# KatherLab/STAMP

Measured on AMD Instinct MI355X. Metric: tiles/sec encoded (224x224, ViT-L/14), higher is better.
Workload: dtype f16

## Files before the change

include/amdstamp.h:

```cpp
#ifndef AMDSTAMP_H
#define AMDSTAMP_H

#include <stddef.h>
#include <stdint.h>

#ifdef __cplusplus
extern "C" {
#endif

#define AMDS_VERSION_MAJOR 0
#define AMDS_VERSION_MINOR 2

typedef enum {
    AMDS_OK = 0,
    AMDS_ERR_INVALID = -1,
    AMDS_ERR_WORKSPACE = -2,
    AMDS_ERR_HIP = -3,
    AMDS_ERR_NODEVICE = -4,
    AMDS_ERR_RANGE = -5
} amds_status;

typedef enum { AMDS_F16 = 0, AMDS_BF16 = 1, AMDS_F32 = 2 } amds_dtype;

typedef enum {
// ... 145 lines not shown

typedef struct {
    const void*  patch_w;
    const float* patch_b;
    const float* prefix;
    const float* pos_patch;
    const amds_vit_block* blocks_host;
    const float* norm_w; const float* norm_b;
    int patch_lo_shift;
    const amds_vit_exact_block* exact_host;
    int exact_hidden;
    const amds_vit_fp8_block* fp8_host;
    const float* pre_norm_w;
    const float* pre_norm_b;
    const amds_vit_exact_block* cls_tail;
} amds_vit_weights;

typedef struct {
    const float* norm1_w; const float* norm1_b;
    const float* qkv_w;   const float* qkv_b;
    const float* proj_w;  const float* proj_b;
    const float* ls1;
    const float* norm2_w; const float* norm2_b;
    const float* fc1_w;   const float* fc1_b;
    const float* fc2_w;   const float* fc2_b;
    const float* ls2;
} amds_vit_host_block;
typedef struct {
    const float* patch_w;
    const float* patch_b;
// ... 24 lines not shown
int amds_vit_forward(const amds_vit_cfg* cfg_host, const amds_vit_weights* w_host,
                     const uint8_t* tiles, void* feats_f16, int B, int chunk,
                     void* ws, size_t ws_bytes, void* stream);

int amds_check_finite(const void* x, long n, int dtype, int* count_dev, int* count_host, void* stream);

int amds_vit_forward_tokens(const amds_vit_cfg* cfg_host, const amds_vit_weights* w_host,
                            const uint8_t* tiles, void* feats_f16, float* tokens_f32, int B, int chunk,
                            void* ws, size_t ws_bytes, void* stream);

int amds_vit_forward_overlapped(amds_ctx* ctx, const amds_vit_cfg* cfg_host, const amds_vit_weights* w_host, const uint8_t* tiles,
                                void* feats_f16, int B, int chunk, void* ws, size_t ws_bytes, void* stream);

int amds_attention_cls_f32(const float* q, long ldq, const void* qkv, float* out, long ldo, int B, int T, int H, int head_dim,
                           int dtype, void* stream);
int amds_vit_cls_gather(const float* x, float* xc, int B, int T, int D, void* stream);
int amds_vit_cls_scatter(const float* xc, float* x, void* xh, float* rowstat, int B, int T, int D, float eps, int dtype, void* stream);
int amds_mlp_act_f32(float* u, long ld, int rows, int hidden, int kind, void* stream);

int amds_tile_im2col_u8(const uint8_t* tiles, void* out, int B, int img, int patch, int kp,
                        int dtype, void* stream);
int amds_tile_im2col_u8_ex(const uint8_t* tiles, void* out, int B, int img, int patch, int kp,
                           int dtype, int lo_shift, void* stream);

int amds_tile_normalize_u8(const uint8_t* hwc, float* chw, int B, int H, int W,
                           const float mean_host[3], const float std_host[3], void* stream);

int amds_tile_edge_fraction_u8(const uint8_t* tiles, float* frac, uint8_t* edges, uint8_t* gray, int B, int S, int low, int high,
                               void* stream);

// ... 647 lines not shown
```

stamp_amd/_lib.py:

```python
from __future__ import annotations

import ctypes as C
import os
from pathlib import Path

LIB_PATH = Path(__file__).resolve().parent / "lib" / "libamdstamp.so"

F16, BF16, F32 = 0, 1, 2
ERR_RANGE = -5
(EPI_BIAS, EPI_BIAS_GELU, EPI_BIAS_RELU, EPI_RESIDUAL, EPI_BIAS_F32, EPI_SWIGLU, EPI_PATCH,
 EPI_BIAS_GELU_F32, EPI_BIAS_RELU_F32) = range(9)


class VitCfg(C.Structure):
    _fields_ = [("img", C.c_int), ("patch", C.c_int), ("dim", C.c_int), ("depth", C.c_int),
                ("heads", C.c_int), ("hidden", C.c_int), ("n_prefix", C.c_int), ("mlp_kind", C.c_int),
                ("layerscale", C.c_int), ("dtype", C.c_int), ("ln_eps", C.c_float)]


class VitBlock(C.Structure):
    _fields_ = [(n, C.c_void_p) for n in (
        "ln1_w", "ln1_b", "qkv_w", "qkv_b", "proj_w", "proj_b", "ls1",
        "ln2_w", "ln2_b", "fc1_w", "fc1_b", "fc2_w", "fc2_b", "ls2", "qkv_colsum", "fc1_colsum")]


class VitExactBlock(C.Structure):
    _fields_ = [(n, C.c_void_p) for n in ("q_w", "q_b", "proj_w", "proj_b", "fc1_w", "fc1_b", "fc2_w", "fc2_b")]


class VitFp8Block(C.Structure):
    _fields_ = ([(n, C.c_void_p) for n in ("qkv_w8", "qkv_cs", "proj_w8", "proj_cs", "proj_b", "fc1_w8", "fc1_cs")] + [("fc1_wnorm_max", C.c_float), ("fc1_babs_max", C.c_float)]
                + [(n, C.c_void_p) for n in ("fc2_w8", "fc2_cs", "fc2_b")])


class VitWeights(C.Structure):
    _fields_ = [("patch_w", C.c_void_p), ("patch_b", C.c_void_p), ("prefix", C.c_void_p),
                ("pos_patch", C.c_void_p), ("blocks_host", C.POINTER(VitBlock)),
                ("norm_w", C.c_void_p), ("norm_b", C.c_void_p), ("patch_lo_shift", C.c_int),
                ("exact_host", C.POINTER(VitExactBlock)), ("exact_hidden", C.c_int), ("fp8_host", C.POINTER(VitFp8Block)),
                ("pre_norm_w", C.c_void_p), ("pre_norm_b", C.c_void_p), ("cls_tail", C.POINTER(VitExactBlock))]


class VitHostBlock(C.Structure):
    _fields_ = [(n, C.c_void_p) for n in ("norm1_w", "norm1_b", "qkv_w", "qkv_b", "proj_w", "proj_b", "ls1", "norm2_w", "norm2_b",
                                          "fc1_w", "fc1_b", "fc2_w", "fc2_b", "ls2")]


class VitHostWeights(C.Structure):
    _fields_ = [("patch_w", C.c_void_p), ("patch_b", C.c_void_p), ("cls_token", C.c_void_p), ("reg_token", C.c_void_p), ("pos_embed", C.c_void_p),
                ("blocks", C.POINTER(VitHostBlock)), ("norm_w", C.c_void_p), ("norm_b", C.c_void_p), ("hidden", C.c_int), ("no_embed_class", C.c_int),
                ("mean", C.c_double * 3), ("std", C.c_double * 3)]


PACK_LNFOLD, PACK_PATCH_SPLIT, PACK_EXACT, PACK_CLS_TAIL = 1, 2, 4, 8

# ... 231 lines not shown
    "amds_swin_forward": (_i, [C.POINTER(SwinCfg), C.POINTER(SwinWeights), _vp, _vp, _vp, _i, _i, _vp, _sz, _vp]),
    "amds_swin_stem": (_i, [_vp, _vp, _vp, _i, _i, _i, _f, _vp]),
    "amds_window_attention": (_i, [_vp, _l, _vp, _l, _vp, _vp, _i, _i, _i, _i, _i, _i, _vp]),
    "amds_swin_attn96": (_i, [_vp, _vp, _vp, _vp, _vp, _vp, _vp, _vp, _vp, _i, _i, _i, _f, _i, _vp]),
    "amds_patch_merge_ln": (_i, [_vp, _vp, _vp, _vp, _i, _i, _i, _f, _i, _vp]),
    "amds_layernorm_meanpool": (_i, [_vp, _vp, _vp, _vp, _vp, _i, _i, _i, _f, _vp]),
    "amds_tile_edge_fraction_u8": (_i, [_vp, _vp, _vp, _vp, _i, _i, _i, _i, _vp]),
    "amds_tile_im2col_u8": (_i, [_vp, _vp, _i, _i, _i, _i, _i, _vp]),
    "amds_tile_im2col_u8_ex": (_i, [_vp, _vp, _i, _i, _i, _i, _i, _i, _vp]),
    "amds_vit_pack_bytes": (_sz, [_vp, _vp, _i]),
    "amds_vit_pack": (_i, [_vp, _vp, _i, _vp, _sz, _vp, _vp, _vp, _vp]),
    "amds_vit_pack_host": (_i, [_vp, _vp, _i, _vp, _sz, _vp, _vp, _vp, _vp]),
    "amds_compact_shift_u8": (_i, [_vp, _vp, _l, _i, _i, _vp, _vp]),
    "amds_compact_rows_u8": (_i, [_vp, _l, _vp, _f, _vp, _i, _vp, _vp, _i, _vp]),
    "amds_attention_cls_f32": (_i, [_vp, _l, _vp, _vp, _l, _i, _i, _i, _i, _i, _vp]),
    "amds_vit_cls_gather": (_i, [_vp, _vp, _i, _i, _i, _vp]),
    "amds_vit_cls_scatter": (_i, [_vp, _vp, _vp, _vp, _i, _i, _i, _f, _i, _vp]),
    "amds_mlp_act_f32": (_i, [_vp, _l, _i, _i, _i, _vp]),
    "amds_tile_normalize_u8": (_i, [_vp, _vp, _i, _i, _i, C.POINTER(_f), C.POINTER(_f), _vp]),
    "amds_macenko_normalize_u8": (_i, [_vp, _vp, _vp, _i, _i, _i, _f, _f, _f, _vp]),
    "amds_supertiles_to_tiles_workspace_bytes": (_sz, [_i, _i, _i, _i]),
    "amds_supertiles_to_tiles_u8": (_i, [_vp, _vp, _i, _i, _i, _i, _vp, _vp, _i, _vp, _sz, _vp]),
    "amds_gather_rows": (_i, [_vp, _l, _vp, _i, _vp, _l, _i, _i, _i, _i, _vp]),
    "amds_vary_precision": (_i, [_vp, _vp, _vp, _l, _i, _vp]),
    "amds_bag_batch_gather": (_i, [_vp, _l, _i, _vp, _vp, _vp, _l, _i, _vp, _i, _i, _i, _i, _u64, _u32, _vp]),
    "amds_bag_batch_shifts": (_i, [_vp, _i, _i, _i, _i, _u64, _u32, _vp]),
    "amds_bag_plan": (_i, [_vp, _vp, _vp, _vp, _i, _i, _u64, _u32, _vp]),
    "amds_mean_pool": (_i, [_vp, _vp, _i, _i, _i, _i, _vp]),
    "amds_linear_f32": (_i, [_vp, _vp, _vp, _vp, _i, _i, _i, _i, _vp]),
    "amds_mil_vit_workspace_bytes": (_sz, [_vp, _i, _i]),
# ... 222 lines not shown
```

stamp_amd/csrc/vit.hip:

```cpp
#include "common.h"

namespace amds {
int prefix_init(const float* prefix, float* x, int B, int T, int P, int dim, hipStream_t st);

struct VitPlan {
    int np, T, kp, dim, hidden;
    size_t off_x, off_h, off_qkv, off_mlp, off_h2, off_lo, off_rowpart, off_rowstat, off_xc, off_hc, off_qc, off_oc, off_uc, off_diag, off_q8, off_q8s, off_q8n, off_q8u, total;
};

static inline size_t align256(size_t v) { return (v + 255) & ~(size_t)255; }

static int make_plan(const amds_vit_cfg* c, int batch, VitPlan* p) {
    AMDS_REQUIRE(c != nullptr, "vit: null cfg");
    AMDS_REQUIRE(c->img > 0 && c->patch > 0 && c->img % c->patch == 0, "vit: img=%d not divisible by patch=%d", c->img, c->patch);
    AMDS_REQUIRE(c->dim % 128 == 0 && c->heads > 0 && (c->heads * 64 == c->dim || c->heads * 80 == c->dim),
                 "vit: dim=%d must be a multiple of 128 and heads*64 or heads*80", c->dim);
    AMDS_REQUIRE(c->hidden % 64 == 0 && c->hidden > 0, "vit: hidden=%d must be a multiple of 64 (zero-pad)", c->hidden);
    AMDS_REQUIRE(c->mlp_kind >= 0 && c->mlp_kind <= 2, "vit: bad mlp_kind");
    AMDS_REQUIRE(c->mlp_kind == 1 || c->hidden % 128 == 0, "vit: GELU hidden=%d must be a multiple of 128", c->hidden);
    AMDS_REQUIRE(c->dtype == AMDS_F16 || c->dtype == AMDS_BF16, "vit: bad act dtype");
    AMDS_REQUIRE(c->depth > 0 && c->n_prefix >= 0 && batch > 0, "vit: bad depth/prefix/batch");
    const int g = c->img / c->patch;
    p->np = g * g;
    p->T = p->np + c->n_prefix;
// ... 67 lines not shown
        for (int l = 0; l < c->depth; ++l)
            AMDS_REQUIRE(ex[l].q_w && ex[l].q_b && ex[l].proj_w && ex[l].proj_b && ex[l].fc1_w && ex[l].fc1_b && ex[l].fc2_w && ex[l].fc2_b &&
                         w->blocks_host[l].ln1_w && w->blocks_host[l].ln1_b && w->blocks_host[l].ln2_w && w->blocks_host[l].ln2_b,
                         "vit: exact block %d: incomplete weights", l);
    }
    const bool tail_env = !(getenv("AMDS_VIT_CLS_TAIL") && atoi(getenv("AMDS_VIT_CLS_TAIL")) == 0);
    const amds_vit_exact_block* tl = (tail_env && tokens_f32 == nullptr && c->mlp_kind != 2) ? (ex ? &ex[c->depth - 1] : w->cls_tail) : nullptr;
    if (tl) {
        AMDS_REQUIRE(xh_ > 0 && xh_ <= Hd && xh_ % 4 == 0, "vit: exact_hidden=%d must be a multiple of 4 and <= hidden=%d", xh_, Hd);
        const amds_vit_block& lb = w->blocks_host[c->depth - 1];
        AMDS_REQUIRE(tl->q_w && tl->q_b && tl->proj_w && tl->proj_b && tl->fc1_w && tl->fc1_b && tl->fc2_w && tl->fc2_b && lb.ln1_w && lb.ln1_b && lb.ln2_w && lb.ln2_b,
                     "vit: cls_tail: incomplete weights");
    }
    const bool planes_env = !(getenv("AMDS_VIT_PLANES") && atoi(getenv("AMDS_VIT_PLANES")) == 0);
    const bool planes = planes_env && fold && !ex && dt == AMDS_F16;
    const amds_vit_fp8_block* f8 = w->fp8_host;
    if (f8) {
        AMDS_REQUIRE(!fold && !ex && dt == AMDS_F16, "vit: the fp8 path needs the plain packing (no LayerNorm fold, no exact rows) and fp16 activations");
        AMDS_REQUIRE(D % 256 == 0 && Hd % 256 == 0, "vit: the fp8 path needs dim %% 256 == 0 and hidden %% 256 == 0");
        for (int l = 0; l < c->depth; ++l)
            AMDS_REQUIRE(f8[l].qkv_w8 && f8[l].qkv_cs && f8[l].proj_w8 && f8[l].proj_cs && f8[l].proj_b && f8[l].fc1_w8 && f8[l].fc1_cs && f8[l].fc2_w8 && f8[l].fc2_cs && f8[l].fc2_b,
                         "vit: fp8 block %d: incomplete weights", l);
    }
    char* q8 = ws + pl.off_q8;
    float* q8s = reinterpret_cast<float*>(ws + pl.off_q8s);
    float* q8n = reinterpret_cast<float*>(ws + pl.off_q8n);
    float* q8u = reinterpret_cast<float*>(ws + pl.off_q8u);
    float* xc = reinterpret_cast<float*>(ws + pl.off_xc);
    float* hc = reinterpret_cast<float*>(ws + pl.off_hc);
    float* qc = reinterpret_cast<float*>(ws + pl.off_qc);
// ... 42 lines not shown
        float *xcq = xc + (size_t)q.t0 * D, *hcq = hc + (size_t)q.t0 * D, *qcq = qc + (size_t)q.t0 * D, *ocq = oc + (size_t)q.t0 * D;
        float* ucq = uc + (size_t)q.t0 * 2 * Hd;
        auto lin32 = [&](const float* A, int lda, const float* Wt, int K, float* Cm, int ldc, int N, const float* bias, int acc) {
            return bgemm_f32_exact(A, lda, 0, 0, Wt, K, 0, 0, 1, Cm, ldc, 0, 0, 1, 1, q.nt, N, K, 1.0f, 0.0f, bias, acc, s);
        };
        if (ex) AMDS_TRY(amds_vit_cls_gather(xq, xcq, q.nt, T, D, s));
        if (planes) AMDS_TRY(amds_ln_stats_split(xq, D, n, D, c->ln_eps, hq, loq, D, rs, s));
        else if (fold) AMDS_TRY(amds_ln_stats_cast(xq, D, n, D, c->ln_eps, hq, D, rs, dt, s));
        for (int l = 0; l < c->depth; ++l) {
            const amds_vit_block& b = w->blocks_host[l];
            const bool last = l + 1 == c->depth;
            const float* ls1 = c->layerscale ? b.ls1 : nullptr;
            const float* ls2 = c->layerscale ? b.ls2 : nullptr;
            if (last && tl) {
                const size_t wkv = (size_t)D * D;
                if (f8) {
                    char* a8 = q8 + (size_t)r0 * (Hd > D ? Hd : D);
                    float* as = q8s + r0;
                    AMDS_TRY(amds_layernorm_quant_e4m3(xq, D, b.ln1_w, b.ln1_b, c->ln_eps, a8, D, as, nullptr, n, D, s));
                    AMDS_TRY(amds_gemm_fp8(a8, D, (const char*)f8[l].qkv_w8 + wkv, D, n, 2 * D, D, AMDS_EPI_BIAS, qkvq + (size_t)D * 2, 3 * D, b.qkv_b + D,
                                           f8[l].qkv_cs + D, as, s));
                } else if (fold) {
                    AMDS_TRY(amds_gemm_lnfold(hq, D, (const char*)b.qkv_w + wkv * 2, D, n, 2 * D, D, dt, AMDS_EPI_BIAS, qkvq + (size_t)D * 2, 3 * D, b.qkv_b + D,
                                              nullptr, nullptr, nullptr, rs, b.qkv_colsum + D, s));
                } else {
                    AMDS_TRY(amds_layernorm(xq, D, b.ln1_w, b.ln1_b, hq, D, n, D, c->ln_eps, dt, s));
                    AMDS_TRY(amds_gemm_ex((3 * D) % 256 == 0 ? kcfg : -1, hq, D, (const char*)b.qkv_w + wkv * 2, D, n, 2 * D, D, dt, AMDS_EPI_BIAS, qkvq + (size_t)D * 2, 3 * D,
                                          b.qkv_b + D, nullptr, nullptr, 0, 0, 0, 1.0f, s));
                }
                if (planes) AMDS_TRY(amds_planes_to_f32(hq, loq, D, T, xcq, D, q.nt, D, s));
                else if (!ex) AMDS_TRY(amds_vit_cls_gather(xq, xcq, q.nt, T, D, s));
                AMDS_TRY(amds_layernorm(xcq, D, b.ln1_w, b.ln1_b, hcq, D, q.nt, D, c->ln_eps, AMDS_F32, s));
                AMDS_TRY(lin32(hcq, D, tl->q_w, D, qcq, D, D, tl->q_b, 0));
                AMDS_TRY(amds_attention_cls_f32(qcq, D, qkvq, ocq, D, q.nt, T, c->heads, hd, dt, s));
                AMDS_TRY(lin32(ocq, D, tl->proj_w, D, xcq, D, D, tl->proj_b, 1));
                AMDS_TRY(amds_layernorm(xcq, D, b.ln2_w, b.ln2_b, hcq, D, q.nt, D, c->ln_eps, AMDS_F32, s));
                AMDS_TRY(lin32(hcq, D, tl->fc1_w, D, ucq, xf1, xf1, tl->fc1_b, 0));
                AMDS_TRY(amds_mlp_act_f32(ucq, xf1, q.nt, xh_, c->mlp_kind, s));
                AMDS_TRY(lin32(ucq, xf1, tl->fc2_w, xh_, xcq, D, D, tl->fc2_b, 1));
                continue;
            }
            if (f8) {
                char* a8 = q8 + (size_t)r0 * (Hd > D ? Hd : D);
                float* as = q8s + r0;
                float *an = q8n + r0, *au = q8u + r0;
                char* u8 = mlp + (size_t)r0 * Hd;
                AMDS_TRY(amds_layernorm_quant_e4m3(xq, D, b.ln1_w, b.ln1_b, c->ln_eps, a8, D, as, nullptr, n, D, s));
                AMDS_TRY(amds_gemm_fp8(a8, D, f8[l].qkv_w8, D, n, 3 * D, D, AMDS_EPI_BIAS, qkvq, 3 * D, b.qkv_b, f8[l].qkv_cs, as, s));
                AMDS_TRY(amds_attention_vit_hd(qkvq, hq, q.nt, T, c->heads, D / c->heads, dt, s));
// ... 194 lines not shown
```

stamp_amd/csrc/vit_pack.hip:

```cpp
#include "common.h"

#include <algorithm>
#include <cmath>
#include <cstdlib>
#include <thread>
#include <vector>

namespace amds {
namespace {

inline uint16_t f32_to_f16_bits(float v) {
    uint32_t u;
    memcpy(&u, &v, 4);
    const uint32_t sign = u & 0x80000000u;
    u ^= sign;
    uint16_t o;
    if (u >= ((127u + 16u) << 23)) {
        o = u > (255u << 23) ? 0x7e00 : 0x7c00;
    } else if (u < (113u << 23)) {
        const uint32_t magic_bits = ((127u - 15u) + (23u - 10u) + 1u) << 23;
        float f, magic;
        memcpy(&f, &u, 4);
        memcpy(&magic, &magic_bits, 4);
        f += magic;
// ... 44 lines not shown
inline size_t up256(size_t v) { return (v + 255) & ~(size_t)255; }

struct Arena {
    char* host;
    char* target;
    size_t off = 0;
    template <typename T> T* take(size_t n, const T** target_ptr) {
        off = up256(off);
        T* h = host ? reinterpret_cast<T*>(host + off) : nullptr;
        if (target_ptr) *target_ptr = reinterpret_cast<const T*>(target + off);
        off += n * sizeof(T);
        return h;
    }
};

struct Dims { int D, P, np, kp, Hp, Hr, fc1_rows_real, fc1_rows_pad, n_pos; bool swiglu, fold, split, exact, tail; int lo_shift; };

int make_dims(const amds_vit_cfg* c, const amds_vit_host_weights* s, int flags, Dims* d) {
    AMDS_REQUIRE(c && s, "amds_vit_pack: null cfg / weights");
    AMDS_REQUIRE(c->img > 0 && c->patch > 0 && c->img % c->patch == 0 && c->dim > 0 && c->depth > 0 && c->n_prefix >= 1, "amds_vit_pack: bad cfg");
    AMDS_REQUIRE(c->dtype == AMDS_F16 || c->dtype == AMDS_BF16, "amds_vit_pack: bad act dtype");
    AMDS_REQUIRE(s->patch_w && s->patch_b && s->cls_token && s->pos_embed && s->blocks && s->norm_w && s->norm_b, "amds_vit_pack: incomplete host weights");
    AMDS_REQUIRE(c->n_prefix == 1 || s->reg_token, "amds_vit_pack: %d prefix tokens but no reg_token", c->n_prefix);
    AMDS_REQUIRE(s->hidden > 0 && s->hidden <= c->hidden && c->hidden % 64 == 0, "amds_vit_pack: hidden=%d must be <= cfg.hidden=%d (the 64-padded width)", s->hidden, c->hidden);
    d->D = c->dim; d->P = c->n_prefix;
    const int g = c->img / c->patch;
    d->np = g * g;
    d->kp = ((3 * c->patch * c->patch + 63) / 64) * 64;
    d->Hp = c->hidden; d->Hr = s->hidden;
    d->swiglu = c->mlp_kind == 1;
    AMDS_REQUIRE(d->swiglu || d->Hr == d->Hp, "amds_vit_pack: a GELU MLP's hidden width (%d) must not need padding (cfg.hidden=%d)", d->Hr, d->Hp);
    d->fc1_rows_real = d->swiglu ? 2 * d->Hr : d->Hr;
    d->fc1_rows_pad = d->swiglu ? 2 * d->Hp : d->Hp;
    d->n_pos = d->np + (s->no_embed_class ? 0 : d->P);
    d->fold = (flags & AMDS_PACK_LNFOLD) != 0;
    d->split = (flags & AMDS_PACK_PATCH_SPLIT) != 0;
    d->exact = (flags & AMDS_PACK_EXACT) != 0;
    d->tail = (flags & AMDS_PACK_CLS_TAIL) != 0 && c->mlp_kind != 2;
    d->lo_shift = d->split ? (c->dtype == AMDS_F16 ? 11 : 8) : 0;
    if (d->fold) AMDS_REQUIRE(d->D % 256 == 0 && d->fc1_rows_pad % 256 == 0, "amds_vit_pack: LayerNorm fold needs dim %% 256 == 0 and fc1 rows %% 256 == 0 (dim=%d, fc1 rows=%d)", d->D, d->fc1_rows_pad);
    AMDS_REQUIRE(!d->swiglu || d->Hp % 32 == 0, "amds_vit_pack: SwiGLU hidden_pad %% 32");
    for (int l = 0; l < c->depth; ++l) {
        const amds_vit_host_block& b = s->blocks[l];
        AMDS_REQUIRE(b.norm1_w && b.norm1_b && b.qkv_w && b.qkv_b && b.proj_w && b.proj_b && b.norm2_w && b.norm2_b && b.fc1_w && b.fc1_b && b.fc2_w && b.fc2_b,
                     "amds_vit_pack: block %d: incomplete host weights", l);
        AMDS_REQUIRE(!c->layerscale || (b.ls1 && b.ls2), "amds_vit_pack: block %d: LayerScale configured but ls1 / ls2 missing", l);
    }
    return AMDS_OK;
}

void pack_linear(const Act16& a, const float* W, const float* bias, int K, const std::vector<int>& row_src, const float* gamma, const float* beta,
                 uint16_t* dst, int ld, float* bias_out, float* colsum_out) {
    const int R = (int)row_src.size();
    for (int r = 0; r < R; ++r) {
// ... 53 lines not shown
    float* prefix = A.take<float>((size_t)d.P * D, ow ? &ow->prefix : nullptr);
    float* posp = A.take<float>((size_t)d.np * D, ow ? &ow->pos_patch : nullptr);
    if (fill) {
        for (int t = 0; t < d.P; ++t)
            for (int k = 0; k < D; ++k) {
                float v = t == 0 ? s->cls_token[k] : s->reg_token[(size_t)(t - 1) * D + k];
                if (!s->no_embed_class) v = v + s->pos_embed[(size_t)t * D + k];
                prefix[(size_t)t * D + k] = v;
            }
        copy_f32(posp, s->pos_embed + (s->no_embed_class ? 0 : (size_t)d.P * D), (size_t)d.np * D);
    }
    float* nw = A.take<float>(D, ow ? &ow->norm_w : nullptr);
    float* nb = A.take<float>(D, ow ? &ow->norm_b : nullptr);
    if (fill) { copy_f32(nw, s->norm_w, D); copy_f32(nb, s->norm_b, D); }
    if (ow) { ow->blocks_host = ob; ow->patch_lo_shift = d.lo_shift; ow->exact_host = d.exact ? oe : nullptr; ow->exact_hidden = d.Hr; ow->fp8_host = nullptr; ow->pre_norm_w = nullptr; ow->pre_norm_b = nullptr;
              ow->cls_tail = d.tail ? &oe[c->depth - 1] : nullptr; }

    std::vector<int> id3(3 * D), idD(D), fc1_map(d.fc1_rows_pad);
    for (int i = 0; i < 3 * D; ++i) id3[i] = i;
    for (int i = 0; i < D; ++i) idD[i] = i;
    if (d.swiglu) {
        for (int r = 0; r < d.fc1_rows_pad; ++r) {
            const int blk = r / 64, w = r % 64, unit = blk * 32 + (w % 32);
            fc1_map[r] = unit < d.Hr ? (w < 32 ? unit : d.Hr + unit) : -1;
        }
    } else {
        for (int r = 0; r < d.fc1_rows_pad; ++r) fc1_map[r] = r;
    }

    struct Slot { uint16_t *qkv, *proj, *fc1, *fc2; float *qkv_b, *qkv_c, *proj_b, *fc1_b, *fc1_c, *fc2_b, *ln1w, *ln1b, *ln2w, *ln2b, *ls1, *ls2;
                  float *xq_w, *xq_b, *xp_w, *xp_b, *x1_w, *x1_b, *x2_w, *x2_b; };
    std::vector<Slot> slots(c->depth);
    for (int l = 0; l < c->depth; ++l) {
        Slot& t = slots[l];
        amds_vit_block* b = ob ? &ob[l] : nullptr;
        const void* q = nullptr;
#define TAKE16(field, n, dst) do { t.field = A.take<uint16_t>((n), reinterpret_cast<const uint16_t**>(&q)); if (b) b->dst = q; } while (0)
#define TAKE32(field, n, dst) t.field = A.take<float>((n), b ? &b->dst : nullptr)
        TAKE32(ln1w, D, ln1_w); TAKE32(ln1b, D, ln1_b);
        TAKE16(qkv, (size_t)3 * D * D, qkv_w); TAKE32(qkv_b, 3 * D, qkv_b);
        TAKE16(proj, (size_t)D * D, proj_w); TAKE32(proj_b, D, proj_b);
        TAKE32(ln2w, D, ln2_w); TAKE32(ln2b, D, ln2_b);
        TAKE16(fc1, (size_t)d.fc1_rows_pad * D, fc1_w); TAKE32(fc1_b, d.fc1_rows_pad, fc1_b);
        TAKE16(fc2, (size_t)D * d.Hp, fc2_w); TAKE32(fc2_b, D, fc2_b);
        if (c->layerscale) { TAKE32(ls1, D, ls1); TAKE32(ls2, D, ls2); }
        else { t.ls1 = t.ls2 = nullptr; if (b) b->ls1 = b->ls2 = nullptr; }
        if (d.fold) { TAKE32(qkv_c, 3 * D, qkv_colsum); TAKE32(fc1_c, d.fc1_rows_pad, fc1_colsum); }
        else { t.qkv_c = t.fc1_c = nullptr; if (b) b->qkv_colsum = b->fc1_colsum = nullptr; }
#undef TAKE16
#undef TAKE32
        t.xq_w = nullptr;
        if (d.exact || (d.tail && l + 1 == c->depth)) {
            amds_vit_exact_block* e = oe ? &oe[l] : nullptr;
            t.xq_w = A.take<float>((size_t)D * D, e ? &e->q_w : nullptr);        t.xq_b = A.take<float>(D, e ? &e->q_b : nullptr);
            t.xp_w = A.take<float>((size_t)D * D, e ? &e->proj_w : nullptr);     t.xp_b = A.take<float>(D, e ? &e->proj_b : nullptr);
            t.x1_w = A.take<float>((size_t)d.fc1_rows_real * D, e ? &e->fc1_w : nullptr); t.x1_b = A.take<float>(d.fc1_rows_real, e ? &e->fc1_b : nullptr);
            t.x2_w = A.take<float>((size_t)D * d.Hr, e ? &e->fc2_w : nullptr);   t.x2_b = A.take<float>(D, e ? &e->fc2_b : nullptr);
        }
    }
    if (!fill) return AMDS_OK;
    auto do_block = [&](int l) {
        const amds_vit_host_block& hb = s->blocks[l];
        const Slot& t = slots[l];
        copy_f32(t.ln1w, hb.norm1_w, D); copy_f32(t.ln1b, hb.norm1_b, D);
        copy_f32(t.ln2w, hb.norm2_w, D); copy_f32(t.ln2b, hb.norm2_b, D);
        if (d.fold) {
            pack_linear(a, hb.qkv_w, hb.qkv_b, D, id3, hb.norm1_w, hb.norm1_b, t.qkv, D, t.qkv_b, t.qkv_c);
            pack_linear(a, hb.fc1_w, hb.fc1_b, D, fc1_map, hb.norm2_w, hb.norm2_b, t.fc1, D, t.fc1_b, t.fc1_c);
        } else {
            pack_linear(a, hb.qkv_w, hb.qkv_b, D, id3, nullptr, nullptr, t.qkv, D, t.qkv_b, nullptr);
            pack_linear(a, hb.fc1_w, hb.fc1_b, D, fc1_map, nullptr, nullptr, t.fc1, D, t.fc1_b, nullptr);
        }
        pack_linear(a, hb.proj_w, hb.proj_b, D, idD, nullptr, nullptr, t.proj, D, t.proj_b, nullptr);
        pack_linear(a, hb.fc2_w, hb.fc2_b, d.Hr, idD, nullptr, nullptr, t.fc2, d.Hp, t.fc2_b, nullptr);
        if (t.ls1) { copy_f32(t.ls1, hb.ls1, D); copy_f32(t.ls2, hb.ls2, D); }
        if (t.xq_w) {
            copy_f32(t.xq_w, hb.qkv_w, (size_t)D * D); copy_f32(t.xq_b, hb.qkv_b, D);
            copy_f32(t.x1_w, hb.fc1_w, (size_t)d.fc1_rows_real * D); copy_f32(t.x1_b, hb.fc1_b, d.fc1_rows_real);
            for (int n = 0; n < D; ++n) {
                const float g1 = hb.ls1 && c->layerscale ? hb.ls1[n] : 1.0f, g2 = hb.ls2 && c->layerscale ? hb.ls2[n] : 1.0f;
                for (int k = 0; k < D; ++k) t.xp_w[(size_t)n * D + k] = hb.proj_w[(size_t)n * D + k] * g1;
                for (int k = 0; k < d.Hr; ++k) t.x2_w[(size_t)n * d.Hr + k] = hb.fc2_w[(size_t)n * d.Hr + k] * g2;
                t.xp_b[n] = hb.proj_b[n] * g1;
                t.x2_b[n] = hb.fc2_b[n] * g2;
            }
        }
    };
    unsigned nthreads = std::min<unsigned>(std::min<unsigned>((unsigned)c->depth, 16u), std::max(1u, std::thread::hardware_concurrency()));
    if (const char* e = getenv("AMDS_PACK_THREADS")) nthreads = std::max(1, atoi(e));
    std::vector<std::thread> pool;
    std::atomic<int> next{0};
    for (unsigned i = 0; i < nthreads; ++i)
        pool.emplace_back([&] { for (int l = next.fetch_add(1); l < c->depth; l = next.fetch_add(1)) do_block(l); });
    for (auto& th : pool) th.join();
    return AMDS_OK;
}

}
}

using namespace amds;
// ... 42 lines not shown
```

stamp_amd/vit.py:

```python
from __future__ import annotations

import ctypes as C
import math
import os
from dataclasses import dataclass, field, replace

import torch
from torch import nn

from . import _lib, ops

IMAGENET_MEAN = (0.485, 0.456, 0.406)
IMAGENET_STD = (0.229, 0.224, 0.225)


@dataclass(frozen=True)
class ViTConfig:
    img: int = 224
    patch: int = 14
    dim: int = 1024
    depth: int = 24
    heads: int = 16
    hidden: int = 4096
    mlp: str = "gelu"
# ... 20 lines not shown
    @property
    def hidden_pad(self) -> int:
        return (self.hidden + 63) // 64 * 64

    @property
    def kp(self) -> int:
        return (3 * self.patch * self.patch + 63) // 64 * 64

    def matmul_flops_per_tile(self) -> float:
        T, D, np_ = self.tokens, self.dim, self.n_patches
        fc1_out = self.hidden * (2 if self.mlp == "swiglu" else 1)
        lin = 2 * T * (D * 3 * D + D * D + D * fc1_out + self.hidden * D)
        att = 2 * 2 * T * T * D
        return 2 * np_ * 3 * self.patch ** 2 * D + self.depth * (lin + att)

    def matmul_flops_skipped_by_cls_tail(self) -> float:
        T, D = self.tokens, self.dim
        fc1_out = self.hidden * (2 if self.mlp == "swiglu" else 1)
        return 2 * (T - 1) * (D * D + D * D + D * fc1_out + self.hidden * D) + 2 * 2 * T * (T - 1) * D


PRESETS: dict[str, ViTConfig] = {
    "vit_large_patch14_224": ViTConfig(),
    "uni2_h": ViTConfig(dim=1536, depth=24, heads=24, hidden=4096, mlp="swiglu", reg_tokens=8, no_embed_class=True),
    "virchow2": ViTConfig(dim=1280, depth=32, heads=16, hidden=3416, mlp="swiglu", reg_tokens=4, no_embed_class=False),
    "virchow": ViTConfig(dim=1280, depth=32, heads=16, hidden=3416, mlp="swiglu", reg_tokens=0, no_embed_class=False),
    "test_tiny_hd80": ViTConfig(dim=640, depth=2, heads=8, hidden=696, mlp="swiglu", reg_tokens=4, no_embed_class=False),
    "h_optimus_0": ViTConfig(dim=1536, depth=40, heads=24, hidden=4096, mlp="swiglu", reg_tokens=4, no_embed_class=True,
                             mean=(0.707223, 0.578729, 0.703617), std=(0.211883, 0.230117, 0.177517)),
    "gigapath": ViTConfig(patch=16, dim=1536, depth=40, heads=24, hidden=4096, mlp="swiglu", reg_tokens=0, no_embed_class=False),
    "dinobloom_s": ViTConfig(dim=384, depth=12, heads=6, hidden=1536),
    "plip": ViTConfig(patch=32, dim=768, depth=12, heads=12, hidden=3072, mlp="quick_gelu", pre_norm=True, layerscale=False, ln_eps=1e-5,
                      mean=(0.48145466, 0.4578275, 0.40821073), std=(0.26862954, 0.26130258, 0.27577711)),
    "vit_large_patch16_224": ViTConfig(patch=16),
# ... 117 lines not shown
        if cls_tail is None:
            cls_tail = os.environ.get("AMDS_VIT_CLS_TAIL", "1") != "0"
        self.cls_tail = bool(cls_tail) and cfg.mlp != "quick_gelu"
        if cfg.mlp == "quick_gelu":
            if exact or fp8 or ln_fold:
                raise ValueError("a quick_gelu (CLIP) trunk runs on the plain packing only: no ln_fold, exact or fp8")
            self.ln_fold = False
        if self.fp8:
            if act_dtype != torch.float16 or exact or cfg.dim % 256 or cfg.hidden % 256 or cfg.mlp == "quick_gelu":
                raise ValueError("fp8=True needs fp16 activations, exact=False, and dim / hidden multiples of 256 (ViT-L, UNI2-h, H-optimus; not Virchow's 3416)")
            self.ln_fold = False
        self._pack(state_dict)
        if self.fp8:
            self._pack_fp8(state_dict)

    def _pack(self, sd: dict[str, torch.Tensor]) -> None:
        c = self.cfg
        validate_state_dict(c, sd)
        hw, keep = host_weights(c, sd)
        flags = (_lib.PACK_LNFOLD if self.ln_fold else 0) | (_lib.PACK_PATCH_SPLIT if self.patch_lo_shift else 0) | (_lib.PACK_EXACT if self.exact else 0) \
            | (_lib.PACK_CLS_TAIL if self.cls_tail else 0)
        self._cfg_c = _lib.VitCfg(c.img, c.patch, c.dim, c.depth, c.heads, c.hidden_pad, c.n_prefix, {"gelu": 0, "swiglu": 1, "quick_gelu": 2}[c.mlp],
                                  1 if c.layerscale else 0, ops.act_code(self.act_dtype), c.ln_eps)
        lib = _lib.lib()
        need = lib.amds_vit_pack_bytes(C.byref(self._cfg_c), C.byref(hw), flags)
        if need == 0:
            _lib.check(-1, "vit_pack_bytes")
        self._image = torch.empty(need, dtype=torch.uint8, device=self.device_)
        self._w_c = _lib.VitWeights()
        self._blocks = (_lib.VitBlock * c.depth)()
# ... 291 lines not shown
```

Before: 6434.

## Fold last-layer K/V projection into CLS-query attention over normalized activations

In the final block's CLS-only tail, the full K/V projection over all tokens is no longer computed. The CLS query is projected through each head's K weights (with the LayerNorm gain folded in), and a streaming kernel takes dot products directly against the fp16 pre-norm activations using per-row statistics and an online softmax. It accumulates the weighted sum of activations, which is then multiplied by the V weights once per tile. This removes a T×D×2D GEMM per tile in the last layer, at the cost of a custom kernel, extra packed weights, and hi/lo fp16 splitting for accuracy.

```diff
diff --git a/include/amdstamp.h b/include/amdstamp.h
--- a/include/amdstamp.h
+++ b/include/amdstamp.h
@@ -183,6 +183,8 @@
     const float* pre_norm_w;
     const float* pre_norm_b;
     const amds_vit_exact_block* cls_tail;
+    const float* cq_kv_w;
+    const float* cq_kv_cs;
 } amds_vit_weights;
 
 typedef struct {
@@ -237,6 +239,9 @@
 
 int amds_attention_cls_f32(const float* q, long ldq, const void* qkv, float* out, long ldo, int B, int T, int H, int head_dim,
                            int dtype, void* stream);
+size_t amds_attention_cls_query_workspace_bytes(int B, int H, int D);
+int amds_attention_cls_query_f32(const float* q, long ldq, const void* xh, long ldx, const float* rowstat, const float* kv_w, const float* kv_cs,
+                                 const float* v_b, float* out, long ldo, int B, int T, int H, int D, void* ws, size_t ws_bytes, void* stream);
 int amds_vit_cls_gather(const float* x, float* xc, int B, int T, int D, void* stream);
 int amds_vit_cls_scatter(const float* xc, float* x, void* xh, float* rowstat, int B, int T, int D, float eps, int dtype, void* stream);
 int amds_mlp_act_f32(float* u, long ld, int rows, int hidden, int kind, void* stream);
diff --git a/stamp_amd/_lib.py b/stamp_amd/_lib.py
--- a/stamp_amd/_lib.py
+++ b/stamp_amd/_lib.py
@@ -38,7 +38,8 @@
                 ("pos_patch", C.c_void_p), ("blocks_host", C.POINTER(VitBlock)),
                 ("norm_w", C.c_void_p), ("norm_b", C.c_void_p), ("patch_lo_shift", C.c_int),
                 ("exact_host", C.POINTER(VitExactBlock)), ("exact_hidden", C.c_int), ("fp8_host", C.POINTER(VitFp8Block)),
-                ("pre_norm_w", C.c_void_p), ("pre_norm_b", C.c_void_p), ("cls_tail", C.POINTER(VitExactBlock))]
+                ("pre_norm_w", C.c_void_p), ("pre_norm_b", C.c_void_p), ("cls_tail", C.POINTER(VitExactBlock)),
+                ("cq_kv_w", C.c_void_p), ("cq_kv_cs", C.c_void_p)]
 
 
 class VitHostBlock(C.Structure):
@@ -300,6 +301,8 @@
     "amds_compact_shift_u8": (_i, [_vp, _vp, _l, _i, _i, _vp, _vp]),
     "amds_compact_rows_u8": (_i, [_vp, _l, _vp, _f, _vp, _i, _vp, _vp, _i, _vp]),
     "amds_attention_cls_f32": (_i, [_vp, _l, _vp, _vp, _l, _i, _i, _i, _i, _i, _vp]),
+    "amds_attention_cls_query_workspace_bytes": (_sz, [_i, _i, _i]),
+    "amds_attention_cls_query_f32": (_i, [_vp, _l, _vp, _l, _vp, _vp, _vp, _vp, _vp, _l, _i, _i, _i, _i, _vp, _sz, _vp]),
     "amds_vit_cls_gather": (_i, [_vp, _vp, _i, _i, _i, _vp]),
     "amds_vit_cls_scatter": (_i, [_vp, _vp, _vp, _vp, _i, _i, _i, _f, _i, _vp]),
     "amds_mlp_act_f32": (_i, [_vp, _l, _i, _i, _i, _vp]),
diff --git a/stamp_amd/csrc/vit.hip b/stamp_amd/csrc/vit.hip
--- a/stamp_amd/csrc/vit.hip
+++ b/stamp_amd/csrc/vit.hip
@@ -105,6 +105,8 @@
     }
     const bool planes_env = !(getenv("AMDS_VIT_PLANES") && atoi(getenv("AMDS_VIT_PLANES")) == 0);
     const bool planes = planes_env && fold && !ex && dt == AMDS_F16;
+    const bool cq_env = !(getenv("AMDS_VIT_CLS_QUERY") && atoi(getenv("AMDS_VIT_CLS_QUERY")) == 0);
+    const bool cq = cq_env && planes && tl && w->cq_kv_w && w->cq_kv_cs && c->heads * 64 == D && 6L * T >= 8L * c->heads;
     const amds_vit_fp8_block* f8 = w->fp8_host;
     if (f8) {
         AMDS_REQUIRE(!fold && !ex && dt == AMDS_F16, "vit: the fp8 path needs the plain packing (no LayerNorm fold, no exact rows) and fp16 activations");
@@ -177,7 +179,8 @@
             const float* ls2 = c->layerscale ? b.ls2 : nullptr;
             if (last && tl) {
                 const size_t wkv = (size_t)D * D;
-                if (f8) {
+                if (cq) {
+                } else if (f8) {
                     char* a8 = q8 + (size_t)r0 * (Hd > D ? Hd : D);
                     float* as = q8s + r0;
                     AMDS_TRY(amds_layernorm_quant_e4m3(xq, D, b.ln1_w, b.ln1_b, c->ln_eps, a8, D, as, nullptr, n, D, s));
@@ -195,7 +198,9 @@
                 else if (!ex) AMDS_TRY(amds_vit_cls_gather(xq, xcq, q.nt, T, D, s));
                 AMDS_TRY(amds_layernorm(xcq, D, b.ln1_w, b.ln1_b, hcq, D, q.nt, D, c->ln_eps, AMDS_F32, s));
                 AMDS_TRY(lin32(hcq, D, tl->q_w, D, qcq, D, D, tl->q_b, 0));
-                AMDS_TRY(amds_attention_cls_f32(qcq, D, qkvq, ocq, D, q.nt, T, c->heads, hd, dt, s));
+                if (cq) AMDS_TRY(amds_attention_cls_query_f32(qcq, D, hq, D, rs, w->cq_kv_w, w->cq_kv_cs, b.qkv_b + 2 * D, ocq, D, q.nt, T, c->heads, D, qkvq,
+                                                              (size_t)n * 3 * D * 2, s));
+                else AMDS_TRY(amds_attention_cls_f32(qcq, D, qkvq, ocq, D, q.nt, T, c->heads, hd, dt, s));
                 AMDS_TRY(lin32(ocq, D, tl->proj_w, D, xcq, D, D, tl->proj_b, 1));
                 AMDS_TRY(amds_layernorm(xcq, D, b.ln2_w, b.ln2_b, hcq, D, q.nt, D, c->ln_eps, AMDS_F32, s));
                 AMDS_TRY(lin32(hcq, D, tl->fc1_w, D, ucq, xf1, xf1, tl->fc1_b, 0));
diff --git a/stamp_amd/csrc/vit_cls_query.hip b/stamp_amd/csrc/vit_cls_query.hip
--- /dev/null
+++ b/stamp_amd/csrc/vit_cls_query.hip
@@ -0,0 +1,211 @@
+#include "common.h"
+
+namespace amds {
+
+constexpr int CQ_ROWS = 16, CQ_HEADS = 16;
+template <int DV>
+__global__ void __launch_bounds__(256, 2) cls_query_stream_kernel(const f16* __restrict__ xh, long ldx, const float* __restrict__ rowstat,
+                                                               const float* __restrict__ tq, const float* __restrict__ q, long ldq,
+                                                               const float* __restrict__ cs_k, const float* __restrict__ cs_v,
+                                                               const float* __restrict__ b_v, float* __restrict__ s_out, float* __restrict__ out,
+                                                               long ldo, int Tn, int H, float scale) {
+    constexpr int D = 256 * DV, LDR = D + 8;
+    constexpr int KS = 2 * DV;
+    constexpr int NLD = 2 * DV;
+    __shared__ __attribute__((aligned(16))) f16 xs[CQ_ROWS * LDR];
+    __shared__ float part[4][CQ_HEADS][CQ_ROWS];
+    __shared__ __attribute__((aligned(16))) float wts[CQ_ROWS][CQ_HEADS];
+    __shared__ __attribute__((aligned(16))) float alpha_s[CQ_HEADS];
+    __shared__ float c_s[CQ_HEADS];
+    typedef f16 vecd __attribute__((ext_vector_type(DV)));
+    const int tid = threadIdx.x, lane = tid & 63, wave = tid >> 6;
+    const int l15 = lane & 15, kq = lane >> 4;
+    const long b = blockIdx.x;
+    const f16* xb = xh + b * Tn * ldx;
+    const float* rsb = rowstat + 2 * b * Tn;
+
+    {
+        const int h = tid >> 4, d0 = (tid & 15) * 4;
+        float c = 0.f;
+        if (h < H) {
+#pragma unroll
+            for (int e = 0; e < 4; ++e) c = fmaf(cs_k[h * 64 + d0 + e], q[b * ldq + h * 64 + d0 + e], c);
+        }
+        c += __shfl_xor(c, 1, 64);
+        c += __shfl_xor(c, 2, 64);
+        c += __shfl_xor(c, 4, 64);
+        c += __shfl_xor(c, 8, 64);
+        if ((tid & 15) == 0) c_s[h] = c;
+    }
+    f16x8 t_hi[KS], t_lo[KS];
+#pragma unroll
+    for (int ks = 0; ks < KS; ++ks) {
+        f32x4 v0 = {0.f, 0.f, 0.f, 0.f}, v1 = v0;
+        if (l15 < H) {
+            const float* tp = tq + (b * H + l15) * D + wave * (D / 4) + ks * 32 + kq * 8;
+            v0 = *reinterpret_cast<const f32x4*>(tp);
+            v1 = *reinterpret_cast<const f32x4*>(tp + 4);
+        }
+#pragma unroll
+        for (int e = 0; e < 4; ++e) {
+            const f16 h0 = (f16)v0[e], h1 = (f16)v1[e];
+            t_hi[ks][e] = h0;
+            t_hi[ks][4 + e] = h1;
+            t_lo[ks][e] = (f16)(v0[e] - (float)h0);
+            t_lo[ks][4 + e] = (f16)(v1[e] - (float)h1);
+        }
+    }
+    u32x4 pre[NLD];
+    auto load_chunk = [&](int r0) {
+#pragma unroll
+        for (int i = 0; i < NLD; ++i) {
+            const int p = tid + 256 * i, row = p / (D / 8), c8 = p % (D / 8);
+            pre[i] = u32x4{0u, 0u, 0u, 0u};
+            if (r0 + row < Tn) pre[i] = *reinterpret_cast<const u32x4*>(xb + (long)(r0 + row) * ldx + c8 * 8);
+        }
+    };
+    float acc[CQ_HEADS][DV];
+#pragma unroll
+    for (int h = 0; h < CQ_HEADS; ++h)
+#pragma unroll
+        for (int v = 0; v < DV; ++v) acc[h][v] = 0.f;
+    float run_m = -INFINITY, run_sum = 0.f, run_a = 0.f;
+    const int sh = tid >> 4, sj = tid & 15;
+
+    load_chunk(0);
+    for (int r0 = 0; r0 < Tn; r0 += CQ_ROWS) {
+        __syncthreads();
+#pragma unroll
+        for (int i = 0; i < NLD; ++i) {
+            const int p = tid + 256 * i, row = p / (D / 8), c8 = p % (D / 8);
+            *reinterpret_cast<u32x4*>(xs + row * LDR + c8 * 8) = pre[i];
+        }
+        __syncthreads();
+        if (r0 + CQ_ROWS < Tn) load_chunk(r0 + CQ_ROWS);
+        f32x4 sc = {0.f, 0.f, 0.f, 0.f};
+#pragma unroll
+        for (int ks = 0; ks < KS; ++ks) {
+            const f16x8 xf = *reinterpret_cast<const f16x8*>(xs + l15 * LDR + wave * (D / 4) + ks * 32 + kq * 8);
+            sc = Act<f16>::mfma16(t_hi[ks], xf, sc);
+            sc = Act<f16>::mfma16(t_lo[ks], xf, sc);
+        }
+#pragma unroll
+        for (int i = 0; i < 4; ++i) part[wave][4 * kq + i][l15] = sc[i];
+        __syncthreads();
+        {
+            const int row = r0 + sj;
+            const bool ok = row < Tn;
+            const float dot = (part[0][sh][sj] + part[1][sh][sj]) + (part[2][sh][sj] + part[3][sh][sj]);
+            f32x2 rs2 = {0.f, 0.f};
+            if (ok) rs2 = *reinterpret_cast<const f32x2*>(rsb + 2 * row);
+            const float s = ok ? scale * fmaf(rs2[0], dot, rs2[1] * c_s[sh]) : -INFINITY;
+            float m = s;
+            m = fmaxf(m, __shfl_xor(m, 1, 64));
+            m = fmaxf(m, __shfl_xor(m, 2, 64));
+            m = fmaxf(m, __shfl_xor(m, 4, 64));
+            m = fmaxf(m, __shfl_xor(m, 8, 64));
+            const float new_m = fmaxf(run_m, m);
+            const float al = expf(run_m - new_m);
+            const float p = expf(s - new_m);
+            float ps = p, pa = p * rs2[1];
+            ps += __shfl_xor(ps, 1, 64);  pa += __shfl_xor(pa, 1, 64);
+            ps += __shfl_xor(ps, 2, 64);  pa += __shfl_xor(pa, 2, 64);
+            ps += __shfl_xor(ps, 4, 64);  pa += __shfl_xor(pa, 4, 64);
+            ps += __shfl_xor(ps, 8, 64);  pa += __shfl_xor(pa, 8, 64);
+            run_sum = fmaf(run_sum, al, ps);
+            run_a = fmaf(run_a, al, pa);
+            run_m = new_m;
+            wts[sj][sh] = p * rs2[0];
+            if (sj == 0) alpha_s[sh] = al;
+        }
+        __syncthreads();
+        {
+            const f32x4* ap = reinterpret_cast<const f32x4*>(alpha_s);
+#pragma unroll
+            for (int g = 0; g < 4; ++g) {
+                const f32x4 a4 = ap[g];
+#pragma unroll
+                for (int e = 0; e < 4; ++e)
+#pragma unroll
+                    for (int v = 0; v < DV; ++v) acc[4 * g + e][v] *= a4[e];
+            }
+            const int nr = Tn - r0 < CQ_ROWS ? Tn - r0 : CQ_ROWS;
+            for (int j = 0; j < nr; ++j) {
+                const vecd xv = *reinterpret_cast<const vecd*>(xs + j * LDR + tid * DV);
+                float xf[DV];
+#pragma unroll
+                for (int v = 0; v < DV; ++v) xf[v] = (float)xv[v];
+                const f32x4* wp = reinterpret_cast<const f32x4*>(&wts[j][0]);
+#pragma unroll
+                for (int g = 0; g < 4; ++g) {
+                    const f32x4 w4 = wp[g];
+#pragma unroll
+                    for (int e = 0; e < 4; ++e)
+#pragma unroll
+                        for (int v = 0; v < DV; ++v) acc[4 * g + e][v] = fmaf(w4[e], xf[v], acc[4 * g + e][v]);
+                }
+            }
+        }
+    }
+    __syncthreads();
+    if (sj == 0) {
+        const float inv = 1.0f / run_sum;
+        alpha_s[sh] = inv;
+        c_s[sh] = run_a * inv;
+    }
+    __syncthreads();
+#pragma unroll
+    for (int h = 0; h < CQ_HEADS; ++h) {
+        if (h < H) {
+            const float inv = alpha_s[h];
+            float* sp = s_out + (b * H + h) * D + tid * DV;
+#pragma unroll
+            for (int v = 0; v < DV; ++v) sp[v] = acc[h][v] * inv;
+        }
+    }
+    for (int i = tid; i < H * 64; i += 256) out[b * ldo + i] = fmaf(cs_v[i], c_s[i >> 6], b_v[i]);
+}
+
+}
+
+using namespace amds;
+
+extern "C" size_t amds_attention_cls_query_workspace_bytes(int B, int H, int D) {
+    if (B <= 0 || H <= 0 || D <= 0) return 0;
+    return 2 * (size_t)B * H * D * sizeof(float);
+}
+
+extern "C" int amds_attention_cls_query_f32(const float* q, long ldq, const void* xh, long ldx, const float* rowstat, const float* kv_w,
+                                            const float* kv_cs, const float* v_b, float* out, long ldo, int B, int T, int H, int D, void* ws,
+                                            size_t ws_bytes, void* stream) {
+    AMDS_REQUIRE(q && xh && rowstat && kv_w && kv_cs && v_b && out && ws, "amds_attention_cls_query_f32: null pointer");
+    AMDS_REQUIRE(B >= 0 && T > 0 && H > 0 && H <= CQ_HEADS && D == H * 64 && (D == 256 || D == 512 || D == 1024),
+                 "amds_attention_cls_query_f32: needs 4, 8 or 16 heads of 64 channels (H=%d, D=%d)", H, D);
+    AMDS_REQUIRE(ldx % 8 == 0 && ldx >= D && ldq >= D && ldo >= D && ldq % 4 == 0 && ldo % 4 == 0, "amds_attention_cls_query_f32: bad pitches");
+    AMDS_REQUIRE((((uintptr_t)xh | (uintptr_t)ws | (uintptr_t)q | (uintptr_t)out | (uintptr_t)kv_w) & 15) == 0 && ((uintptr_t)rowstat & 7) == 0,
+                 "amds_attention_cls_query_f32: pointers must be 16-byte aligned (rowstat: 8)");
+    AMDS_REQUIRE(ws_bytes >= amds_attention_cls_query_workspace_bytes(B, H, D), "amds_attention_cls_query_f32: workspace too small");
+    if (B == 0) return AMDS_OK;
+    hipStream_t st = (hipStream_t)stream;
+    float* tq = reinterpret_cast<float*>(ws);
+    float* sb = tq + (size_t)B * H * D;
+    const float* wk = kv_w;
+    const float* wv = kv_w + (size_t)D * D;
+    int rc;
+    rc = bgemm_f32_exact(q, (int)ldq, 0, 64, wk, D, 0, (long)64 * D, 0, tq, H * D, 0, D, 1, H, B, D, 64, 1.0f, 0.0f, nullptr, 0, stream);
+    if (rc != AMDS_OK) return rc;
+    {
+        ProfScope prof(PROF_ATTN, 2.0 * 2.0 * (double)B * T * H * D, st);
+        const float scale = 0.125f;
+#define AMDS_CQ(DV_) hipLaunchKernelGGL((cls_query_stream_kernel<DV_>), dim3(B), dim3(256), 0, st, (const f16*)xh, ldx, rowstat, tq, q, ldq, kv_cs, kv_cs + D, v_b, \
+                                        sb, out, ldo, T, H, scale)
+        switch (D / 256) {
+            case 1: AMDS_CQ(1); break;
+            case 2: AMDS_CQ(2); break;
+            default: AMDS_CQ(4); break;
+        }
+#undef AMDS_CQ
+        AMDS_LAUNCH_CHECK("cls_query_stream_kernel");
+    }
+    return bgemm_f32_exact(sb, H * D, 0, D, wv, D, 0, (long)64 * D, 1, out, (int)ldo, 0, 64, 1, H, B, 64, D, 1.0f, 0.0f, nullptr, 1, stream);
+}
diff --git a/stamp_amd/csrc/vit_pack.hip b/stamp_amd/csrc/vit_pack.hip
--- a/stamp_amd/csrc/vit_pack.hip
+++ b/stamp_amd/csrc/vit_pack.hip
@@ -82,7 +82,7 @@
     }
 };
 
-struct Dims { int D, P, np, kp, Hp, Hr, fc1_rows_real, fc1_rows_pad, n_pos; bool swiglu, fold, split, exact, tail; int lo_shift; };
+struct Dims { int D, P, np, kp, Hp, Hr, fc1_rows_real, fc1_rows_pad, n_pos; bool swiglu, fold, split, exact, tail, cq; int lo_shift; };
 
 int make_dims(const amds_vit_cfg* c, const amds_vit_host_weights* s, int flags, Dims* d) {
     AMDS_REQUIRE(c && s, "amds_vit_pack: null cfg / weights");
@@ -106,6 +106,7 @@
     d->exact = (flags & AMDS_PACK_EXACT) != 0;
     d->tail = (flags & AMDS_PACK_CLS_TAIL) != 0 && c->mlp_kind != 2;
     d->lo_shift = d->split ? (c->dtype == AMDS_F16 ? 11 : 8) : 0;
+    d->cq = d->tail && d->fold && c->dtype == AMDS_F16 && c->heads * 64 == d->D && (d->D == 256 || d->D == 512 || d->D == 1024);
     if (d->fold) AMDS_REQUIRE(d->D % 256 == 0 && d->fc1_rows_pad % 256 == 0, "amds_vit_pack: LayerNorm fold needs dim %% 256 == 0 and fc1 rows %% 256 == 0 (dim=%d, fc1 rows=%d)", d->D, d->fc1_rows_pad);
     AMDS_REQUIRE(!d->swiglu || d->Hp % 32 == 0, "amds_vit_pack: SwiGLU hidden_pad %% 32");
     for (int l = 0; l < c->depth; ++l) {
@@ -189,7 +190,7 @@
     float* nb = A.take<float>(D, ow ? &ow->norm_b : nullptr);
     if (fill) { copy_f32(nw, s->norm_w, D); copy_f32(nb, s->norm_b, D); }
     if (ow) { ow->blocks_host = ob; ow->patch_lo_shift = d.lo_shift; ow->exact_host = d.exact ? oe : nullptr; ow->exact_hidden = d.Hr; ow->fp8_host = nullptr; ow->pre_norm_w = nullptr; ow->pre_norm_b = nullptr;
-              ow->cls_tail = d.tail ? &oe[c->depth - 1] : nullptr; }
+              ow->cls_tail = d.tail ? &oe[c->depth - 1] : nullptr; ow->cq_kv_w = nullptr; ow->cq_kv_cs = nullptr; }
 
     std::vector<int> id3(3 * D), idD(D), fc1_map(d.fc1_rows_pad);
     for (int i = 0; i < 3 * D; ++i) id3[i] = i;
@@ -204,7 +205,7 @@
     }
 
     struct Slot { uint16_t *qkv, *proj, *fc1, *fc2; float *qkv_b, *qkv_c, *proj_b, *fc1_b, *fc1_c, *fc2_b, *ln1w, *ln1b, *ln2w, *ln2b, *ls1, *ls2;
-                  float *xq_w, *xq_b, *xp_w, *xp_b, *x1_w, *x1_b, *x2_w, *x2_b; };
+                  float *xq_w, *xq_b, *xp_w, *xp_b, *x1_w, *x1_b, *x2_w, *x2_b, *cq_w, *cq_cs; };
     std::vector<Slot> slots(c->depth);
     for (int l = 0; l < c->depth; ++l) {
         Slot& t = slots[l];
@@ -232,6 +233,11 @@
             t.x1_w = A.take<float>((size_t)d.fc1_rows_real * D, e ? &e->fc1_w : nullptr); t.x1_b = A.take<float>(d.fc1_rows_real, e ? &e->fc1_b : nullptr);
             t.x2_w = A.take<float>((size_t)D * d.Hr, e ? &e->fc2_w : nullptr);   t.x2_b = A.take<float>(D, e ? &e->fc2_b : nullptr);
         }
+        t.cq_w = nullptr;
+        if (d.cq && l + 1 == c->depth) {
+            t.cq_w = A.take<float>((size_t)2 * D * D, ow ? &ow->cq_kv_w : nullptr);
+            t.cq_cs = A.take<float>((size_t)2 * D, ow ? &ow->cq_kv_cs : nullptr);
+        }
     }
     if (!fill) return AMDS_OK;
     auto do_block = [&](int l) {
@@ -260,6 +266,18 @@
                 t.x2_b[n] = hb.fc2_b[n] * g2;
             }
         }
+        if (t.cq_w) {
+            for (int r = 0; r < 2 * D; ++r) {
+                const float* wrow = hb.qkv_w + (size_t)(D + r) * D;
+                float* drow = t.cq_w + (size_t)r * D;
+                double cs = 0.0;
+                for (int k = 0; k < D; ++k) {
+                    drow[k] = (float)((double)wrow[k] * (double)hb.norm1_w[k]);
+                    cs += (double)drow[k];
+                }
+                t.cq_cs[r] = (float)cs;
+            }
+        }
     };
     unsigned nthreads = std::min<unsigned>(std::min<unsigned>((unsigned)c->depth, 16u), std::max(1u, std::thread::hardware_concurrency()));
     if (const char* e = getenv("AMDS_PACK_THREADS")) nthreads = std::max(1, atoi(e));
diff --git a/stamp_amd/vit.py b/stamp_amd/vit.py
--- a/stamp_amd/vit.py
+++ b/stamp_amd/vit.py
@@ -58,10 +58,13 @@
         att = 2 * 2 * T * T * D
         return 2 * np_ * 3 * self.patch ** 2 * D + self.depth * (lin + att)
 
-    def matmul_flops_skipped_by_cls_tail(self) -> float:
+    def matmul_flops_skipped_by_cls_tail(self, cls_query: bool = False) -> float:
         T, D = self.tokens, self.dim
         fc1_out = self.hidden * (2 if self.mlp == "swiglu" else 1)
-        return 2 * (T - 1) * (D * D + D * D + D * fc1_out + self.hidden * D) + 2 * 2 * T * (T - 1) * D
+        skipped = 2 * (T - 1) * (D * D + D * D + D * fc1_out + self.hidden * D) + 2 * 2 * T * (T - 1) * D
+        if cls_query:
+            skipped += 2 * T * 2 * D * D - 2 * 2 * D * D - 2 * 2 * T * self.heads * D + 2 * 2 * T * D
+        return skipped
 
 
 PRESETS: dict[str, ViTConfig] = {
@@ -209,6 +212,16 @@
         if self.fp8:
             self._pack_fp8(state_dict)
 
+    @property
+    def cls_query(self) -> bool:
+        planes = self.ln_fold and not self.exact and not self.fp8 and self.act_dtype == torch.float16 and os.environ.get("AMDS_VIT_PLANES", "1") != "0"
+        return (bool(self._w_c.cq_kv_w) and planes and self.cls_tail and os.environ.get("AMDS_VIT_CLS_TAIL", "1") != "0"
+                and os.environ.get("AMDS_VIT_CLS_QUERY", "1") != "0")
+
+    def matmul_flops_executed_per_tile(self) -> float:
+        skipped = self.cfg.matmul_flops_skipped_by_cls_tail(cls_query=self.cls_query) if self.cls_tail and os.environ.get("AMDS_VIT_CLS_TAIL", "1") != "0" else 0.0
+        return self.cfg.matmul_flops_per_tile() - skipped
+
     def _pack(self, sd: dict[str, torch.Tensor]) -> None:
         c = self.cfg
         validate_state_dict(c, sd)
```

Result: no change. 6461, median of 6 (+0.4%).
